# RGenomicsETL/duckhts

Hardware: AMD Instinct MI355X
Metric: read_bam_records_per_sec (higher is better)
Workload: dtype u8

## Files before the change

### duckhts_amd/__init__.py

```python
import ctypes as C
import os

import numpy as np

_HERE = os.path.dirname(os.path.abspath(__file__))
LIB_PATH = os.environ.get("DHTS_LIB") or os.path.join(_HERE, "libduckhts_amd.so")
_LIB = None

BAM_COLUMNS = ["QNAME", "FLAG", "RNAME", "POS", "MAPQ", "CIGAR", "RNEXT", "PNEXT", "TLEN", "SEQ", "QUAL",
               "READ_GROUP_ID", "SAMPLE_ID"]
K_NAMES = ["sigscan", "huff_decode", "lz_resolve", "tiles", "core_unpack", "scan", "string_write", "bcf_check", "bcf_measure", "bcf_write"]


class StrCol(C.Structure):
    _fields_ = [("off", C.c_void_p), ("len", C.c_void_p), ("bytes", C.c_void_p), ("nbytes", C.c_uint64)]


class BamBatch(C.Structure):
    _fields_ = [("n_rows", C.c_int64), ("status", C.c_int32), ("seq_packed", C.c_int32),
                ("flag", C.c_void_p), ("pos", C.c_void_p), ("mapq", C.c_void_p), ("pnext", C.c_void_p),
                ("tlen", C.c_void_p), ("tid", C.c_void_p), ("mtid", C.c_void_p), ("rg_idx", C.c_void_p),
                ("rg_valid", C.c_void_p),
                ("qname", StrCol), ("cigar", StrCol), ("seq", StrCol), ("qual", StrCol), ("rg", StrCol),
                ("first_rec_uoff", C.c_uint64), ("end_uoff", C.c_uint64), ("n_tag_cols", C.c_int32), ("qual_bits", C.c_int32), ("aux_map", C.c_void_p), ("tag_cols", C.c_void_p),
# ... 139 lines not shown
           "dhts_udf_upload", "dhts_udf_apply", "dhts_udf_result_host_bytes", "dhts_udf_fetch", "dhts_udf_seq_kmers", "dhts_udf_kmers_host_bytes", "dhts_udf_kmers_fetch"]


def lib():
    global _LIB
    if _LIB is None:
        if not os.path.exists(LIB_PATH):
            raise RuntimeError(f"{LIB_PATH} is missing: build it with __graft_entry__.build() (hipcc, gfx950)")
        L = C.CDLL(LIB_PATH)
        L.dhts_create.restype = C.c_void_p
        L.dhts_create.argtypes = [C.c_int]
        L.dhts_destroy.argtypes = [C.c_void_p]
        L.dhts_error.restype = C.c_char_p
        L.dhts_error.argtypes = [C.c_void_p]
        L.dhts_open_path.argtypes = [C.c_void_p, C.c_char_p]
        L.dhts_open_host.argtypes = [C.c_void_p, C.c_void_p, C.c_uint64]
        L.dhts_open_tiled.argtypes = [C.c_void_p, C.c_void_p, C.c_uint64, C.c_void_p, C.c_uint64, C.c_int, C.c_void_p,
                                      C.c_uint64]
        L.dhts_resident_bytes.restype = C.c_uint64
        L.dhts_resident_bytes.argtypes = [C.c_void_p]
        L.dhts_bgzf_index.restype = C.c_int64
        L.dhts_bgzf_index.argtypes = [C.c_void_p]
        L.dhts_bgzf_table.argtypes = [C.c_void_p, C.c_void_p, C.c_void_p, C.c_void_p, C.c_int64]
        L.dhts_bgzf_inflate_to_host.restype = C.c_int64
        L.dhts_bgzf_inflate_to_host.argtypes = [C.c_void_p, C.c_int64, C.c_int64, C.c_void_p, C.c_uint64, C.c_void_p]
        L.dhts_bam_open.argtypes = [C.c_void_p]
        L.dhts_bam_header_get.argtypes = [C.c_void_p, C.POINTER(BamHeader)]
        L.dhts_bam_is_text.argtypes = [C.c_void_p]
        L.dhts_debug_sam_records.restype = C.c_int64
        L.dhts_debug_sam_records.argtypes = [C.c_void_p, C.c_void_p, C.c_uint64, C.POINTER(C.c_int64)]
        L.dhts_debug_fastq_records.restype = C.c_int64
        L.dhts_debug_fastq_records.argtypes = [C.c_void_p, C.c_void_p, C.c_uint64, C.POINTER(C.c_int64)]
        L.dhts_debug_tile_stats.argtypes = [C.c_void_p, C.POINTER(C.c_uint64)]
        L.dhts_bam_set_shard.argtypes = [C.c_void_p, C.c_int, C.c_int]
        L.dhts_bam_set_block_range.argtypes = [C.c_void_p, C.c_int64, C.c_int64, C.c_int]
        L.dhts_shard_cut.argtypes = [C.c_void_p, C.c_int64, C.c_uint64, C.c_int, C.c_int, C.POINTER(C.c_int64), C.POINTER(C.c_int64)]
        L.dhts_bam_rewind.argtypes = [C.c_void_p]
        L.dhts_bam_set_regions.argtypes = [C.c_void_p, C.c_char_p]
        L.dhts_bam_std_tag_info.argtypes = [C.c_int, C.c_char_p, C.c_char_p, C.c_char_p]
        L.dhts_bam_set_tag_columns.argtypes = [C.c_void_p, C.c_void_p, C.c_int32]
        L.dhts_bam_set_aux_map.argtypes = [C.c_void_p, C.c_int, C.c_int]
        L.dhts_bam_build_index.restype = C.c_int64
        L.dhts_bam_build_index.argtypes = [C.c_void_p]
        L.dhts_bam_index_bytes.argtypes = [C.c_void_p, C.c_void_p, C.c_uint64]
        L.dhts_bam_set_overlap_intervals.argtypes = [C.c_void_p, C.c_void_p, C.c_void_p, C.c_void_p, C.c_int64]
        L.dhts_bam_load_index.argtypes = [C.c_void_p, C.c_void_p, C.c_uint64]
        L.dhts_bam_next_batch.argtypes = [C.c_void_p, C.c_int64, C.c_uint32, C.POINTER(BamBatch)]
        L.dhts_memcpy_d2h.argtypes = [C.c_void_p, C.c_void_p, C.c_void_p, C.c_uint64]
        L.dhts_sync.argtypes = [C.c_void_p]
        L.dhts_kernel_time_ms.restype = C.c_double
        L.dhts_kernel_time_ms.argtypes = [C.c_void_p, C.c_int, C.POINTER(C.c_int64)]
        L.dhts_kernel_time_reset.argtypes = [C.c_void_p]
        L.dhts_set_timing.argtypes = [C.c_void_p, C.c_int]
        L.dhts_bcf_open.argtypes = [C.c_void_p, C.c_int]
        L.dhts_bcf_info_get.argtypes = [C.c_void_p, C.POINTER(BcfInfo)]
        L.dhts_bcf_set_projection.argtypes = [C.c_void_p, C.c_void_p, C.c_int32]
        L.dhts_bcf_set_block_range.argtypes = [C.c_void_p, C.c_int64, C.c_int64, C.c_int]
        L.dhts_bcf_rewind.argtypes = [C.c_void_p]
        L.dhts_bcf_set_region.argtypes = [C.c_void_p, C.c_char_p]
        L.dhts_bcf_load_index.argtypes = [C.c_void_p, C.c_void_p, C.c_uint64]
        L.dhts_bcf_next_batch.argtypes = [C.c_void_p, C.c_int64, C.POINTER(BcfBatch)]
        L.dhts_fasta_build_index.restype = C.c_int64
        L.dhts_fasta_build_index.argtypes = [C.c_void_p]
        L.dhts_fasta_index_bytes.argtypes = [C.c_void_p, C.c_void_p, C.c_uint64]
        L.dhts_fasta_gzi_bytes.restype = C.c_int64
        L.dhts_fasta_gzi_bytes.argtypes = [C.c_void_p, C.c_void_p, C.c_uint64]
# ... 153 lines not shown
        coff = np.zeros(n, np.uint64)
        clen = np.zeros(n, np.uint32)
        isize = np.zeros(n, np.uint32)
        st = self.L.dhts_bgzf_table(self.h, coff.ctypes.data, clen.ctypes.data, isize.ctypes.data, n)
        return coff, clen, isize, st

    def bgzf_inflate(self, blk0, nblk, cap):
        out = np.zeros(max(cap, 1), np.uint8)
        st = np.zeros(max(nblk, 1), np.int32)
        n = self._chk(self.L.dhts_bgzf_inflate_to_host(self.h, blk0, nblk, out.ctypes.data, cap, st.ctypes.data))
        return out[:n], st[:nblk]

    def bam_open(self):
        self._chk(self.L.dhts_bam_open(self.h))
        return self.header()

    def bam_is_text(self):
        return self.L.dhts_bam_is_text(self.h)

    def debug_sam_records(self):
        n = C.c_int64(0)
        size = self._chk(self.L.dhts_debug_sam_records(self.h, None, 0, C.byref(n)))
        buf = np.zeros(max(size, 1), np.uint8)
        self._chk(self.L.dhts_debug_sam_records(self.h, buf.ctypes.data, size, C.byref(n)))
        return buf[:size].tobytes(), n.value

    TILE_STATS = ("repaired_tiles", "repair_rounds", "fallback_batches", "spec_retries", "validate_rejections", "gave_up")

    def debug_tile_stats(self):
        out = (C.c_uint64 * 8)()
        self._chk(self.L.dhts_debug_tile_stats(self.h, out))
        return {k: int(out[i]) for i, k in enumerate(self.TILE_STATS)}

    def debug_fastq_records(self):
        n = C.c_int64(0)
        size = self._chk(self.L.dhts_debug_fastq_records(self.h, None, 0, C.byref(n)))
        buf = np.zeros(max(size, 1), np.uint8)
        self._chk(self.L.dhts_debug_fastq_records(self.h, buf.ctypes.data, size, C.byref(n)))
        return buf[:size].tobytes(), n.value

    def debug_deflate_codes(self, counts, maxbits):
        cnt = np.ascontiguousarray(counts, dtype=np.uint32)
        assert cnt.ndim == 2
        lens, codes = np.zeros(cnt.shape, np.uint8), np.zeros(cnt.shape, np.uint32)
        f = self.L.dhts_debug_deflate_codes
        f.argtypes = [C.c_void_p, C.c_void_p, C.c_uint32, C.c_uint32, C.c_int64, C.c_void_p, C.c_void_p]
        self._chk(f(self.h, cnt.ctypes.data, cnt.shape[1], maxbits, cnt.shape[0], lens.ctypes.data, codes.ctypes.data))
        return lens, codes

    def header(self):
        h = BamHeader()
        self._chk(self.L.dhts_bam_header_get(self.h, C.byref(h)))
        return {
            "n_ref": h.n_ref,
            "ref_names": [h.ref_name[i] for i in range(h.n_ref)],
            "ref_len": [h.ref_len[i] for i in range(h.n_ref)],
            "text": C.string_at(h.text, h.l_text) if h.l_text else b"",
            "rg_id": [h.rg_id[i] for i in range(h.n_rg)],
            "rg_sm": [h.rg_sm[i] for i in range(h.n_rg)],
            "first_rec_uoff": h.first_rec_uoff,
        }

    def set_shard(self, rank, world):
        self._chk(self.L.dhts_bam_set_shard(self.h, rank, world))

    def set_block_range(self, b0, b1, speculative):
# ... 1404 lines not shown
```

### duckhts_amd/csrc/bam_tiles_lds.hip

```cpp
#pragma once

#ifndef TL_TILE
#define TL_TILE 8192u
#endif
#define TL_RECS (TL_TILE / 32u)
#define TL_HALO 1024u
#define TR_F_ROWS 1ull
#define TR_F_HEAP 2ull
#define TR_F_TIMEOUT 4ull

struct GSrc {
    typedef uint64_t off;
    const uint8_t *g;
    static __device__ __forceinline__ uint64_t none() { return NONE64; }
    __device__ __forceinline__ uint64_t lim(const BamStream &st) const { return st.ulen; }
    __device__ __forceinline__ uint64_t abs(uint64_t o) const { return o; }
    __device__ __forceinline__ uint8_t u8(uint64_t o) const { return g[o]; }
    __device__ __forceinline__ uint32_t u32(uint64_t o) const { return ldu32(g + o); }
    __device__ __forceinline__ uint64_t u64(uint64_t o) const { uint64_t v; __builtin_memcpy(&v, g + o, 8); return v; }
};
struct LSrc { const uint8_t *g; const uint8_t *l; uint64_t base; uint32_t len; };

struct PSrc {
    typedef uint64_t off;
// ... 283 lines not shown
            while (rel < lim) {
                if (rel + 4u > win) { general = true; break; }
                uint32_t v; __builtin_memcpy(&v, buf + rel, 4);
                const int32_t b = (int32_t)__builtin_amdgcn_readfirstlane((int)v);
                if (b < 32) { err = 1; break; }
                if (left - rel - 4u < (uint32_t)b) { if (st.final_batch) err = 1; break; }
                if (lane == 0 && cnt < TL_RECS) rl[cnt] = (uint16_t)rel;
                cnt++; rel += 4u + (uint32_t)b;
            }
#endif
            o = tb + rel;
            if (general && err == 0) {
                while (o < te) {
                    uint32_t bl = 0;
                    const int rc = ((o - tb) + 64 <= (uint64_t)s.len) ? rec_hop_uniform(st, ls, o, lane, bl) : rec_hop(st, gs, o, bl);
                    if (rc == REC_INCOMPLETE) { if (st.final_batch && o < st.ulen) err = 1; break; }
                    if (rc == REC_INVALID) { err = 1; break; }
                    if (lane == 0 && cnt < TL_RECS) rl[cnt] = (uint16_t)(o - tb);
                    cnt++; o += 4ull + bl;
                }
            }
        }
        en = o;
    } else if (first != NONE64) en = first;
    if (lane == 0) {
        out.first[t] = (first != NONE64 && first < te) ? first : NONE64;
        out.end_next[t] = en; out.count[t] = cnt; out.err[t] = err;
        tile_recs_first[t] = (first != NONE64 && first < te) ? first : NONE64;
    }
    __syncthreads();
    for (uint32_t k = lane; k < cnt && k < TL_RECS; k += 64) tile_recs[(size_t)t * TL_RECS + k] = rl[k];
}

extern "C" __global__ void __launch_bounds__(64)
bam_spec_next(BamStream st, uint64_t from, SpecSkip sk, uint64_t *out) {
    const int lane = threadIdx.x;
    GSrc gs; gs.g = st.u;
    uint64_t first = NONE64;
    for (uint64_t base = from & ~63ull; base < st.ulen; base += 64) {
        const uint64_t o = base + (uint64_t)lane;
        bool ok = false;
        if (o < st.ulen && o >= from) {
            RecInfo r;
            if (rec_check_t(st, gs, o, r, false) == REC_OK) {
                ok = true;
                uint64_t o2 = o + 4ull + r.block_len;
                for (int k = 0; k < 2 && ok; k++) {
                    RecInfo r2;
                    const int rc = rec_check_t(st, gs, o2, r2, false);
                    if (rc == REC_INVALID) ok = false;
                    else if (rc == REC_INCOMPLETE) break;
                    else o2 += 4ull + r2.block_len;
                }
                if (ok && spec_skipped(sk, o)) ok = false;
            }
        }
        const uint64_t m = __ballot(ok);
        if (m) { first = base + (uint64_t)(__ffsll((unsigned long long)m) - 1); break; }
    }
    if (lane == 0) *out = first;
}

struct DictG { const uint32_t *off; const uint8_t *bytes; int32_t n; };
struct DictL { const uint32_t *off; const uint8_t *bytes; int32_t n; };
#define RGL_N 32
#define RGL_BYTES 256
// ... 412 lines not shown
```

### duckhts_amd/csrc/dhts_api.hip

```cpp
#include "../../include/duckhts_amd.h"
#include "bgzf_inflate.hip"
#include "bgzf_huff_wave.hip"
#include "bam_records.hip"
#include "bam_tiles_lds.hip"
#include "bam_tile_rows.hip"
#include "bcf_records.hip"
#include "vcf_text.hip"
#include "bed_text.hip"
#include "tabix_text.hip"
#include "sam_text.hip"
#include "fastq_text.hip"
#include "fasta_index.hip"
#include "fasta_nuc.hip"
#include "seq_udf.hip"
#include "bam_bins.hip"
#include "bam_bedcov.hip"
#include "gzip_serial.hip"
#include "bam_tags.hip"
#include "bgzf_deflate.hip"
#include "hts_index.hip"
#include "bcf_header.h"

#include <errno.h>
#include <time.h>
// ... 191 lines not shown
    uint32_t s_patch_cap = 0;
    int64_t s_last_nrec = 0; uint64_t s_last_len = 0;
    int fastq = 0;
    FastaState fa;
    BedState bed;
    NucState nuc;
    BinsState bins;
    BedcovState cov;
    UdfState udf;
    TabixState tbx;
    bool text_any = false;
    DevBuf f_len, f_flag, f_psum, f_rank, f_mark, f_next, f_plus, f_exit, f_entry, f_stop, f_isstart, f_recrank, f_recline;
    DevBuf v_pos_hi;
    DevBuf v_keep, v_endsv; uint64_t proj_gen = 1, keep_gen = 0; int32_t keep_none = 0, fmt_none = 0; bool keep_all = true, fmt_keep_all = true; DevBuf v_fkeep;
    DevBuf v_cnt, v_base, v_line_off, v_rec_len, v_out, v_ctr, v_undef, v_patch, vd_ctg_off, vd_ctg_bytes, vd_ctg_id, vd_id_off, vd_id_bytes, vd_id_id, vd_id_typ, vd_id_ftyp, vd_ctg_hash, vd_id_hash, v_tok_off, v_tok_bytes, v_tok_bits;
    uint32_t v_undef_cap = 65536, v_patch_cap = 1u << 20;
    uint32_t vd_ctg_hmask = 0, vd_id_hmask = 0;
    bool cache_hit = false; std::string pending_tag;
    std::thread stager; StageProg *prog = nullptr; bool growing = false; uint64_t stage_total = 0;
    uint64_t debug_full_len = 0; bool debug_prefix = false;
    DevBuf spec_skip[SPEC_LISTS];
    uint64_t tile_stats[8] = {0, 0, 0, 0, 0, 0, 0, 0};
    int64_t n_blocks = 0; int bgzf_status = 0;
    DevBuf coff, clen, isize, uoff, blk_status;
    std::vector<uint64_t> h_coff, h_uoff; std::vector<uint32_t> h_clen, h_isize;
    DevBuf lit, tok, meta;
    DevBuf stg_lit, stg_tok, wave_ctr;
    DevBuf wg_lit[2], wg_tok[2], stg2_lit, stg2_tok;
    DevBuf blk_off; bool huff_packed = false;
    int64_t isize_repaired = 0;
    bool pool_full_pending = false;
    int64_t pool_per_block = 65536 + 4096;
    DevBuf sg_cnt, sg_base, sg_cand, sg_hits;
    std::vector<uint8_t> built_index; DevBuf ix_end; BamStream last_stream;
    bool ov_active = false; int64_t ov_n = 0;
    DevBuf ov_beg, ov_end, ov_pmax, ov_bmax, ov_id, ov_first, ov_cnt, ov_off, ov_ids;
    int64_t huff_b0 = 0, huff_nb = 0;
    int64_t wave_slots = 0;
    int64_t super_blocks = 524288;
    DevBuf ubuf[2]; int ucur = 0; uint64_t carry_len = 0;
    DevBuf t_first, t_end, t_count, t_err, t_rowbase, d_res, d_nfixed, d_bstat, t_recs, t_recs_first;
    DevBuf t2_first, t2_end, t2_count, t2_err;
    DevBuf t_look; int64_t rows_slots = 0, rows_hint = 0; uint64_t heap_hint[5] = {0, 0, 0, 0, 0};
    DevBuf c_rgflag;
    DevBuf rec_off, c_flag, c_pos, c_mapq, c_pnext, c_tlen, c_tid, c_mtid, c_rgidx, c_rgvalid;
    DevBuf l_qname, l_cigar, l_seq, l_qual, l_rg, cig_rel, ncig_eff, rg_rel, alen_qual;
    DevBuf o_qname, o_cigar, o_seq, o_qual, o_rg, scan_partial, scan_total;
    DevBuf a_qname, a_cigar, a_seq, a_qual, a_rg;
    bool bam_open = false;
    std::vector<std::string> ref_name; std::vector<const char *> ref_name_p; std::vector<uint32_t> ref_len;
    std::string text;
    std::vector<std::string> rg_id, rg_sm; std::vector<char> rg_has_sm; std::vector<const char *> rg_id_p, rg_sm_p;
    uint64_t first_rec_uoff = 0;
    DevBuf d_rg_off, d_rg_bytes;
    std::vector<int32_t> tag_sel; std::vector<dhts_col> tag_out;
    bool aux_on = false, aux_excl_std = false; dhts_aux_map aux_out;
    DevBuf x_excl, x_valid, x_le, x_lp, x_oe, x_op, x_key, x_kind, x_sub, x_payoff, x_payload;
    DevBuf t_codes, t_dir, t_lens, t_offs, t_partial, t_total, t_coldev, t_fixed, t_valid, t_var;
    bool rg_active = false, rg_all = false, rg_nocoor = false;
    std::vector<int64_t> rg_beg, rg_end; std::vector<uint32_t> rg_tid_first;
    DevBuf d_rg_beg, d_rg_end, d_rg_first, c_keep, c_rowmap;
    bool rg_empty_window = false;
    struct ScanWin { int64_t b0, b1; uint64_t first_uoff, end_uoff; };
    std::vector<ScanWin> wins; size_t win_cur = 0; uint64_t scan_end_uoff = ~0ull;
    uint64_t scan_first_uoff = 0;
    bool bcf_open = false; bool bcf_tidy_req = false;
    dhts::BcfHeader bh; dhts::BcfSchema bsch;
// ... 115 lines not shown
        const bool cclean = hipStreamSynchronize(c->copy_stream) == hipSuccess;
        std::lock_guard<std::mutex> lk(g_cs_mu);
        static bool cs_at_exit = false;
        if (!cs_at_exit) { cs_at_exit = true; std::atexit([]() { std::lock_guard<std::mutex> lk2(g_cs_mu); for (auto &x : g_cs) { if (hipSetDevice(x.dev) != hipSuccess) continue; for (int k = 0; k < 2; k++) { (void)hipEventDestroy(x.snap[k]); (void)hipEventDestroy(x.done[k]); } (void)hipStreamDestroy(x.s); } g_cs.clear(); }); }
        if (cclean && g_cs.size() < 32) g_cs.push_back({c->device, c->copy_stream, {c->ev_snap[0], c->ev_snap[1]}, {c->ev_done[0], c->ev_done[1]}});
        else { for (int k = 0; k < 2; k++) { (void)hipEventDestroy(c->ev_snap[k]); (void)hipEventDestroy(c->ev_done[k]); } (void)hipStreamDestroy(c->copy_stream); }
        c->copy_stream = nullptr;
    }
    bool kept = false;
    if (clean) {
        std::lock_guard<std::mutex> lk(g_ss_mu);
        static bool at_exit = false;
        if (!at_exit) { at_exit = true; std::atexit([]() { std::lock_guard<std::mutex> lk2(g_ss_mu); for (auto &x : g_ss) { if (hipSetDevice(x.dev) != hipSuccess) continue; (void)hipEventDestroy(x.ev); (void)hipStreamDestroy(x.sb); (void)hipStreamDestroy(x.s); } g_ss.clear(); }); }
        if (g_ss.size() < 32) { g_ss.push_back({c->device, c->stream, c->stream_b, c->pf_done}); kept = true; }
    }
    if (!kept) { (void)hipEventDestroy(c->pf_done); (void)hipStreamDestroy(c->stream_b); (void)hipStreamDestroy(c->stream); }
    delete c;
}

const char *dhts_error(const dhts_ctx *c) { return c ? c->err.c_str() : "no context (no MI355X device or code object)"; }

static void stop_stager(dhts_ctx *c) {
    if (c->prog && c->stager.joinable()) c->prog->cancel.store(true);
    if (c->stager.joinable()) c->stager.join();
    if (c->prog && !c->pending_tag.empty() && c->prog->finished && c->prog->rc == 0 && c->prog->frontier == c->prog->len) { c->comp.tag = c->pending_tag; c->comp.tag_len = c->prog->len; }
    c->pending_tag.clear();
    delete c->prog; c->prog = nullptr; c->growing = false;
}
static void reset_file_state(dhts_ctx *c) {
    stop_stager(c);
    c->huff_b0 = c->huff_nb = 0; c->file_off = 0; c->file_size = 0; c->seg_split = 0; c->seg_file_off = 0; c->partial_tail = false; c->segs.clear(); c->cache_hit = false; c->gz_plain = c->gz_error = false; c->gz_len = 0; c->plain_text = false; c->vcf_text = false; c->sam_text = false; c->fastq = 0; c->fa.text_ready = false; c->nuc.open = false; c->bins.open = false; c->cov.open = false; c->text_any = false; c->bed.open = false; c->tbx.open = false;
    c->n_blocks = 0; c->bgzf_status = 0; c->bam_open = false; c->range_cut = false; c->last_batch_rows = -1; c->carry_len = 0; c->next_block = 0; c->stream_done = false; c->first_batch = true;
    memset(c->tile_stats, 0, sizeof(c->tile_stats));
    c->h_coff.clear(); c->h_clen.clear(); c->h_isize.clear(); c->h_uoff.clear();
}

int dhts_open_host(dhts_ctx *c, const void *bytes, uint64_t n) {
    if (c) discard_prefetch(c);
    if (!c) return -1;
    HIPCHK(c, hipSetDevice(c->device));
    reset_file_state(c);
    ENSURE(c, c->comp, n + PAD_BYTES);
    HIPCHK(c, hipMemcpyAsync(c->comp.p, bytes, n, hipMemcpyHostToDevice, c->stream));
    HIPCHK(c, hipMemsetAsync((uint8_t *)c->comp.p + n, 0, PAD_BYTES, c->stream));
    HIPCHK(c, hipStreamSynchronize(c->stream));
    c->comp_len = n;
    return 0;
}

int dhts_open_tiled(dhts_ctx *c, const void *head, uint64_t n_head, const void *body, uint64_t n_body, int reps, const void *tail, uint64_t n_tail) {
    if (c) discard_prefetch(c);
    if (!c) return -1;
    HIPCHK(c, hipSetDevice(c->device));
    reset_file_state(c);
    uint64_t n = n_head + n_body * (uint64_t)reps + n_tail;
    ENSURE(c, c->comp, n + PAD_BYTES);
    uint8_t *d = (uint8_t *)c->comp.p;
    if (n_head) HIPCHK(c, hipMemcpyAsync(d, head, n_head, hipMemcpyHostToDevice, c->stream));
    if (n_body && reps > 0) {
        HIPCHK(c, hipMemcpyAsync(d + n_head, body, n_body, hipMemcpyHostToDevice, c->stream));
        for (int r = 1; r < reps; r++) HIPCHK(c, hipMemcpyAsync(d + n_head + n_body * (uint64_t)r, d + n_head, n_body, hipMemcpyDeviceToDevice, c->stream));
    }
    if (n_tail) HIPCHK(c, hipMemcpyAsync(d + n_head + n_body * (uint64_t)reps, tail, n_tail, hipMemcpyHostToDevice, c->stream));
    HIPCHK(c, hipMemsetAsync(d + n, 0, PAD_BYTES, c->stream));
    HIPCHK(c, hipStreamSynchronize(c->stream));
    c->comp_len = n;
// ... 26 lines not shown
```

### duckhts_amd/csrc/dhts_bam_scan.inc

```
struct Batch {
    int64_t b0 = 0, nb = 0; bool in_halo = false, last_of_stream = false, sharded_tail = false, final_batch = false;
    uint64_t carry = 0, ulen = 0, out_base = 0; uint8_t *u = nullptr; int blk_err = 0;
    bool status_pending = false;
};
static const uint32_t NONE32 = 0xffffffffu;
static int batch_begin(dhts_ctx *c, int64_t max_blocks, Batch &B, bool defer = false) {
    if (max_blocks <= 0) max_blocks = 16384;
    if (max_blocks > 24576) max_blocks = 24576;
    B.sharded_tail = (c->shard_b1 < c->n_blocks);
    int64_t b0 = c->next_block;
    int64_t limit = c->shard_b1;
    bool in_halo = b0 >= c->shard_b1;
    if (in_halo) limit = c->n_blocks;
    int64_t nb = limit - b0; if (nb > max_blocks) nb = max_blocks;
    if (in_halo && nb > 4) nb = 4;
    if (nb < 0) nb = 0;
    if (c->first_batch && c->shard_rank != 0 && !in_halo) {
        while (b0 + nb < limit && c->h_uoff[b0 + nb] - c->h_uoff[b0] < (1u << 20) && nb < 24576) nb++;
    }
    B.b0 = b0; B.nb = nb; B.in_halo = in_halo;
    B.last_of_stream = (b0 + nb >= c->n_blocks) && !c->growing;
    {
        const int64_t ahead0 = c->shard_b1 + 8 < c->n_blocks ? c->shard_b1 + 8 : c->n_blocks;
        if (!(c->pf.valid && c->pf.b0 == b0 && c->pf.nb == nb) && huff_ensure(c, b0, nb, ahead0)) return -1;
// ... 192 lines not shown
        int32_t status = 0;
        if (batch_end(c, B, carry_start, false, false, &status)) return -1;
        if (status == 1) break;
        if (status < 0) { rc = -1; err = "the BGZF stream ended on an error"; break; }
    }
    discard_prefetch(c);
    c->next_block = 0; c->carry_len = 0; c->stream_done = false; c->first_batch = true; c->ucur = 0;
    if (rc) return fail(c, "tabix_index: %s", err.c_str());
    if (!inited) init_index();
    uint64_t fin = c->comp_len;
    for (int64_t k = nb; k > 0 && c->h_isize[k - 1] == 0; k--) fin = c->h_coff[k - 1];
    if (!ib.finish(fin << 16)) return fail(c, "tabix_index: %s", ib.err.c_str());
    {
        const uint32_t conf[6] = {(uint32_t)preset, (uint32_t)sc, (uint32_t)bc, (uint32_t)ec, (uint32_t)meta_char, (uint32_t)line_skip}; uint32_t l_nm = 0;
        for (auto &x : names) l_nm += (uint32_t)x.size() + 1;
        auto w32 = [&](uint32_t x) { for (int k = 0; k < 4; k++) ib.aux.push_back((uint8_t)(x >> (8 * k))); };
        for (uint32_t x : conf) w32(x);
        w32(l_nm);
        for (auto &x : names) { ib.aux.insert(ib.aux.end(), x.begin(), x.end()); ib.aux.push_back(0); }
    }
    ib.save(c->built_index);
    return (int64_t)c->built_index.size();
}

extern "C" int dhts_debug_tile_stats(dhts_ctx *c, uint64_t out[8]) {
    if (!c || !out) return -1;
    memcpy(out, c->tile_stats, sizeof(c->tile_stats));
    return 0;
}

static bool rows_deferred_on() { static const bool on = !(getenv("DHTS_ROWS") && !strcmp(getenv("DHTS_ROWS"), "sync")); return on; }
static bool rows_fused_on() { static const bool on = getenv("DHTS_ROWS") && !strcmp(getenv("DHTS_ROWS"), "fused"); return on; }
static int rows_exp() { static const int e = getenv("DHTS_ROWS_EXP") ? (atoi(getenv("DHTS_ROWS_EXP")) & 2) : 0; return e; }
struct RowsQueued { BamCols bc; RowsStr so; };
static int rows_queue(dhts_ctx *c, const BamStream &st, int64_t ntiles, const TileOut &to, uint32_t colmask, RowsQueued &rq) {
    const uint64_t ulen = st.ulen;
    int64_t rcap = (int64_t)(ulen / 160) + 4096; if (c->rows_hint > rcap) rcap = c->rows_hint;
    const uint64_t guess[5] = {ulen / 8 + 65536, ulen / 16 + 65536, ulen / 2 + 65536, ulen / 2 + 65536, ulen / 16 + 65536};
    const uint32_t str_cols = (1u << DHTS_BAM_QNAME) | (1u << DHTS_BAM_CIGAR) | (1u << DHTS_BAM_SEQ) | (1u << DHTS_BAM_QUAL) | (1u << DHTS_BAM_READ_GROUP_ID);
    const bool strings = (colmask & str_cols) != 0;
    const uint32_t hbit[5] = {1u << DHTS_BAM_QNAME, 1u << DHTS_BAM_CIGAR, 1u << DHTS_BAM_SEQ, 1u << DHTS_BAM_QUAL, 1u << DHTS_BAM_READ_GROUP_ID};
    RowsCaps caps; caps.rows = rcap;
    DevBuf *arena[5] = {&c->a_qname, &c->a_cigar, &c->a_seq, &c->a_qual, &c->a_rg};
    for (int k = 0; k < 5; k++) {
        uint64_t want = 0;
        if (colmask & hbit[k]) { want = guess[k]; if (c->heap_hint[k] > want) want = c->heap_hint[k]; }
        if (want) { ENSURE(c, *arena[k], want + PAD_BYTES); caps.heap[k] = arena[k]->cap - PAD_BYTES; } else caps.heap[k] = 0;
    }
    const size_t n = (size_t)rcap;
    ENSURE(c, c->rec_off, n * 4 + 16); ENSURE(c, c->c_rgflag, n + 64);
    ENSURE(c, c->c_flag, n * 2 + 16); ENSURE(c, c->c_pos, n * 8); ENSURE(c, c->c_mapq, n * 4); ENSURE(c, c->c_pnext, n * 8); ENSURE(c, c->c_tlen, n * 8);
    ENSURE(c, c->c_tid, n * 4); ENSURE(c, c->c_mtid, n * 4); ENSURE(c, c->c_rgidx, n * 4); ENSURE(c, c->c_rgvalid, (n / 64 + 2) * 8);
    ENSURE(c, c->l_qname, n * 4 + 16); ENSURE(c, c->l_cigar, n * 4 + 16); ENSURE(c, c->l_seq, n * 4 + 16); ENSURE(c, c->l_qual, n * 4 + 16); ENSURE(c, c->l_rg, n * 4 + 16);
    ENSURE(c, c->cig_rel, n * 4); ENSURE(c, c->ncig_eff, n * 4); ENSURE(c, c->rg_rel, n * 4); ENSURE(c, c->alen_qual, n * 4);
    ENSURE(c, c->o_qname, (n + 1) * 4 + 16); ENSURE(c, c->o_cigar, (n + 1) * 4 + 16); ENSURE(c, c->o_seq, (n + 1) * 4 + 16); ENSURE(c, c->o_qual, (n + 1) * 4 + 16); ENSURE(c, c->o_rg, (n + 1) * 4 + 16);
    BamDict dict; dict.n_rg = (int32_t)c->rg_id.size(); dict.rg_off = (const uint32_t *)c->d_rg_off.p; dict.rg_bytes = (const uint8_t *)c->d_rg_bytes.p; { size_t tb_ = 0; for (auto &id_ : c->rg_id) tb_ += id_.size(); dict.n_bytes = (int32_t)tb_; }
    BamCols &bc = rq.bc; memset(&bc, 0, sizeof(bc));
    bc.flag = (uint16_t *)c->c_flag.p; bc.pos = (int64_t *)c->c_pos.p; bc.mapq = (int32_t *)c->c_mapq.p; bc.pnext = (int64_t *)c->c_pnext.p;
    bc.tlen = (int64_t *)c->c_tlen.p; bc.tid = (int32_t *)c->c_tid.p; bc.mtid = (int32_t *)c->c_mtid.p; bc.rg_idx = (int32_t *)c->c_rgidx.p;
    bc.rg_valid = (uint64_t *)c->c_rgvalid.p; bc.len_qname = (uint32_t *)c->l_qname.p; bc.len_cigar = (uint32_t *)c->l_cigar.p; bc.len_seq = (uint32_t *)c->l_seq.p;
    bc.len_qual = (uint32_t *)c->l_qual.p; bc.len_rg = (uint32_t *)c->l_rg.p; bc.cig_rel = (uint32_t *)c->cig_rel.p; bc.ncig_eff = (uint32_t *)c->ncig_eff.p; bc.rg_rel = (uint32_t *)c->rg_rel.p;
    RowsStr &so = rq.so; memset(&so, 0, sizeof(so));
    so.off[0] = (uint32_t *)c->o_qname.p; so.off[1] = (uint32_t *)c->o_cigar.p; so.off[2] = (uint32_t *)c->o_seq.p; so.off[3] = (uint32_t *)c->o_qual.p; so.off[4] = (uint32_t *)c->o_rg.p;
    for (int k = 0; k < 5; k++) so.heap[k] = (uint8_t *)arena[k]->p;
    so.alen_qual = (uint32_t *)c->alen_qual.p;
    if (c->seq_packed && (colmask & (1u << DHTS_BAM_SEQ))) { ENSURE(c, c->seq_chars, n * 4 + 64); so.seq_chars = (uint32_t *)c->seq_chars.p; }
// ... 96 lines not shown
    ENSURE(c, c->t_rowbase, ntiles * 4 + 16); ENSURE(c, c->d_res, 256); ENSURE(c, c->d_nfixed, 64);
    ENSURE(c, c->t_recs, (size_t)ntiles * TL_RECS * 2 + 64); ENSURE(c, c->t_recs_first, ntiles * 8 + 64);
    ENSURE(c, c->t2_first, ntiles * 8); ENSURE(c, c->t2_end, ntiles * 8); ENSURE(c, c->t2_count, ntiles * 4); ENSURE(c, c->t2_err, ntiles * 4);
    TileOut to; to.first = (uint64_t *)c->t_first.p; to.end_next = (uint64_t *)c->t_end.p; to.count = (uint32_t *)c->t_count.p; to.err = (int32_t *)c->t_err.p;
    TileOut to2; to2.first = (uint64_t *)c->t2_first.p; to2.end_next = (uint64_t *)c->t2_end.p; to2.count = (uint32_t *)c->t2_count.p; to2.err = (int32_t *)c->t2_err.p;
    uint64_t start0;
    if (c->sam_text) start0 = 0;
    else if (c->first_batch) start0 = (c->shard_rank == 0) ? c->scan_first_uoff - out_base : NONE64;
    else start0 = 0;
    if (!c->sam_text && c->first_batch && c->shard_rank == 0 && c->scan_first_uoff < out_base) return fail(c, "internal: header beyond first batch");
    uint64_t res[4] = {0, 0, 0, 0};
    uint64_t first0 = NONE64;
    const bool speculative = (start0 == NONE64);
    const bool fused = !speculative && !(c->rg_active && !c->rg_all) && !(sharded_tail && out_base + ulen > c->h_uoff[c->shard_b1]) && rows_deferred_on();
    unsigned long long hres[16] = {0}; RowsQueued rq;
    uint64_t spec_from = 0, en0 = NONE64; int spec_tries = 0; bool restoring = false;
    SpecSkip sk; memset(&sk, 0, sizeof(sk));
    int status_attempt = 0;
    for (;;) {
        uint64_t start_eff = start0;
        if (speculative && !restoring && spec_tries > 0) {
            uint64_t *d_cand = (uint64_t *)c->d_nfixed.p + 2, cand = NONE64;
            hipLaunchKernelGGL(bam_spec_next, dim3(1), dim3(64), 0, c->stream, st, spec_from, sk, d_cand);
            HIPCHK(c, hipMemcpyAsync(&cand, d_cand, 8, hipMemcpyDeviceToHost, c->stream));
            HIPCHK(c, hipStreamSynchronize(c->stream));
            if (cand == NONE64) { spec_from = 0; restoring = true; c->tile_stats[DHTS_TS_GAVE_UP]++; }
            else { start_eff = cand; c->tile_stats[DHTS_TS_RETRIES]++; }
        }
        to.first = (uint64_t *)c->t_first.p; to.end_next = (uint64_t *)c->t_end.p; to.count = (uint32_t *)c->t_count.p; to.err = (int32_t *)c->t_err.p;
        to2.first = (uint64_t *)c->t2_first.p; to2.end_next = (uint64_t *)c->t2_end.p; to2.count = (uint32_t *)c->t2_count.p; to2.err = (int32_t *)c->t2_err.p;
        uint32_t nfh[2] = {0, 0}, bst[4] = {NONE32, 0, NONE32, 0};
        {
            KTimer tm(c, DHTS_K_TILES);
            hipLaunchKernelGGL(bam_tile_scan, dim3((unsigned)ntiles), dim3(64), 0, c->stream, st, start_eff, ntiles, to, (uint16_t *)c->t_recs.p, (uint64_t *)c->t_recs_first.p, spec_from);
            uint32_t *nf = (uint32_t *)c->d_nfixed.p;
            (void)hipMemsetAsync(nf, 0, 8, c->stream);
            for (int r = 0; r < 2; r++) {
                hipLaunchKernelGGL(bam_tile_fix, dim3((unsigned)((ntiles + 255) / 256)), dim3(256), 0, c->stream, st, TILE_BYTES, ntiles, to, to2, nf + r);
                TileOut tmp = to; to = to2; to2 = tmp;
            }
            hipLaunchKernelGGL(bam_tile_finalize, dim3(1), dim3(1024), 0, c->stream, ntiles, to, (uint32_t *)c->t_rowbase.p, (uint64_t *)c->d_res.p);
        }
        if (fused) { if (rows_queue(c, st, ntiles, to, colmask, rq)) return -1; HIPCHK(c, hipMemcpyAsync(hres, c->d_res.p, 128, hipMemcpyDeviceToHost, c->stream)); }
        HIPCHK(c, hipMemcpyAsync(res, c->d_res.p, 32, hipMemcpyDeviceToHost, c->stream));
        HIPCHK(c, hipMemcpyAsync(&first0, to.first, 8, hipMemcpyDeviceToHost, c->stream));
        if (speculative) HIPCHK(c, hipMemcpyAsync(&en0, to.end_next, 8, hipMemcpyDeviceToHost, c->stream));
        HIPCHK(c, hipMemcpyAsync(nfh, c->d_nfixed.p, 8, hipMemcpyDeviceToHost, c->stream));
        if (B.status_pending) HIPCHK(c, hipMemcpyAsync(bst, c->d_bstat.p, 16, hipMemcpyDeviceToHost, c->stream));
        HIPCHK(c, hipStreamSynchronize(c->stream));
        if (B.status_pending) {
            const int rs = batch_status_resolve(c, B, bst, status_attempt++);
            if (rs < 0) return -1;
            if (rs > 0) {
                ulen = B.ulen; final_batch = B.final_batch;
                st.ulen = ulen; st.final_batch = final_batch ? 1 : 0; c->last_stream = st;
                ntiles = (int64_t)((ulen + TILE_BYTES - 1) / TILE_BYTES); if (ntiles < 1) ntiles = 1;
                spec_from = 0; spec_tries = 0; restoring = false; sk.lists = 0;
                continue;
            }
        }
        if (g_debug) fprintf(stderr, "[dhts] tiles=%lld nfixed=%u,%u\n", (long long)ntiles, nfh[0], nfh[1]);
        c->tile_stats[DHTS_TS_REPAIRED] += (uint64_t)nfh[0] + nfh[1]; c->tile_stats[DHTS_TS_ROUNDS] += (nfh[0] != 0) + (nfh[1] != 0);
        if (nfh[1] != 0) {
            KTimer tm(c, DHTS_K_TILES);
            int rounds = 2; bool seq_fallback = false;
            for (;;) {
                (void)hipMemsetAsync(c->d_nfixed.p, 0, 4, c->stream);
// ... 285 lines not shown
```

### duckhts_amd/csrc/dhts_regions.inc

```
static long long parse_decimal_sep(const char *str, const char **strend) {
    unsigned long long n = 0; int digits = 0, decimals = 0, e = 0; char sign = '+', esign = '+';
    const char *s = str;
    while (*s == ' ' || (*s >= '\t' && *s <= '\r')) s++;
    if (*s == '+' || *s == '-') sign = *s++;
    while (*s) { if (*s >= '0' && *s <= '9') { digits++; n = n * 10 + (unsigned)(*s++ - '0'); } else if (*s == ',') s++; else break; }
    if (*s == '.') { s++; while (*s >= '0' && *s <= '9') { decimals++; digits++; n = n * 10 + (unsigned)(*s++ - '0'); } }
    switch (*s) {
    case 'e': case 'E': s++; if (*s == '+' || *s == '-') esign = *s++; while (*s >= '0' && *s <= '9') e = e * 10 + (*s++ - '0'); if (esign == '-') e = -e; break;
    case 'k': case 'K': e += 3; s++; break;
    case 'm': case 'M': e += 6; s++; break;
    case 'g': case 'G': e += 9; s++; break;
    }
    e -= decimals;
    while (e > 0) { n *= 10; e--; }
    while (e < 0) { n /= 10; e++; }
    *strend = digits > 0 ? s : str;
    return sign == '+' ? (long long)n : -(long long)n;
}

static bool parse_region_token_fn(const std::function<int(const std::string &)> &getid, const std::string &tok, int &tid, int64_t &beg, int64_t &end);
static bool parse_region_token(const std::vector<std::string> &names, const std::string &tok, int &tid, int64_t &beg, int64_t &end) {
    return parse_region_token_fn([&](const std::string &nm) -> int { for (size_t i = 0; i < names.size(); i++) if (names[i] == nm) return (int)i; return -1; }, tok, tid, beg, end);
}
static bool parse_region_token_fn(const std::function<int(const std::string &)> &getid, const std::string &tok, int &tid, int64_t &beg, int64_t &end) {
// ... 360 lines not shown
        all.any = true;
        for (auto &x : merged_windows(w, true)) all.chunks.push_back(x);
    }
    (void)dhts_bcf_set_region(c, nullptr);
    if (whole) return 0;
    std::vector<std::pair<uint64_t, uint64_t>> sg;
    if (all.any) {
        std::sort(all.chunks.begin(), all.chunks.end());
        std::vector<std::pair<uint64_t, uint64_t>> mg;
        const uint64_t gap_bytes = (uint64_t)(getenv("DHTS_WINDOW_GAP_MB") ? atof(getenv("DHTS_WINDOW_GAP_MB")) : 32.0) * (1u << 20);
        for (auto &x : all.chunks) {
            if (!mg.empty() && (x.first >> 16) <= (mg.back().second >> 16) + gap_bytes) { if (x.second > mg.back().second) mg.back().second = x.second; }
            else mg.push_back(x);
        }
        for (auto &x : mg) sg.push_back({x.first >> 16, x.second >> 16});
    }
    *count = (int64_t)sg.size();
    if ((int64_t)sg.size() > cap) { *count = -1; return 0; }
    for (size_t k = 0; k < sg.size(); k++) { beg[k] = sg[k].first; end[k] = sg[k].second; }
    return 0;
}

static void enter_window(dhts_ctx *c, size_t k) {
    const dhts_ctx::ScanWin &w = c->wins[k];
    c->win_cur = k; c->shard_b0 = w.b0; c->shard_b1 = w.b1; c->shard_rank = 0; c->shard_world = (w.b1 < c->n_blocks) ? 2 : 1;
    c->scan_first_uoff = w.first_uoff; c->scan_end_uoff = w.end_uoff;
}
int dhts_bam_rewind(dhts_ctx *c) {
    if (!c) return -1;
    discard_prefetch(c);
    if (!c->wins.empty()) enter_window(c, 0);
    c->next_block = c->shard_b0; c->carry_len = 0; c->stream_done = c->rg_empty_window; c->first_batch = true; c->ucur = 0;
    c->huff_b0 = c->huff_nb = 0;
    memset(c->tile_stats, 0, sizeof(c->tile_stats));
    skip_header_blocks(c);
    return 0;
}
```

### include/duckhts_amd_debug.h

```cpp
#ifndef DUCKHTS_AMD_DEBUG_H
#define DUCKHTS_AMD_DEBUG_H
#include "duckhts_amd.h"
#ifdef __cplusplus
extern "C" {
#endif

void dhts_debug_malloc_stats(uint64_t *calls, uint64_t *bytes, double *seconds);
int64_t dhts_debug_index_prefix(dhts_ctx *, uint64_t nbytes);
int64_t dhts_debug_vcf_records(dhts_ctx *, uint8_t *dst, uint64_t cap, uint32_t *rec_off, int64_t nrec);
int64_t dhts_debug_sam_records(dhts_ctx *, uint8_t *dst, uint64_t cap, int64_t *nrec);
int64_t dhts_debug_fastq_records(dhts_ctx *, uint8_t *dst, uint64_t cap, int64_t *nrec);
int64_t dhts_debug_bed_walk(dhts_ctx *, double *ms_line_table, double *ms_walk);
void dhts_debug_bedcov_max_rows(uint64_t n);
double dhts_debug_time_huff(dhts_ctx *, int64_t b0, int64_t nb, int reps);
double dhts_debug_time_lz(dhts_ctx *, int64_t b0, int64_t nb, int reps);
int dhts_debug_huff_run(dhts_ctx *, int64_t b0, int64_t nb, int kernel);
int dhts_debug_scratch_get(dhts_ctx *, int64_t s, uint32_t *meta4, uint8_t *lit, uint32_t *tok);
int dhts_debug_meta(dhts_ctx *, int64_t s, uint32_t *out4);
int dhts_debug_deflate_codes(dhts_ctx *, const uint32_t *counts, uint32_t nsym, uint32_t maxbits, int64_t ncases, uint8_t *lens_out, uint32_t *codes_out);
int dhts_debug_tile_stats(dhts_ctx *, uint64_t out[8]);
int dhts_debug_diag(dhts_ctx *, unsigned long long *out8);
int dhts_debug_hw_diag(dhts_ctx *, unsigned long long *out16, int reset);
int dhts_debug_tr_diag(dhts_ctx *, unsigned long long *out16, int reset);

#ifdef __cplusplus
}
#endif
#endif
```

Baseline: 614.6 million.

## Add one-thread-per-tile BAM tile scan kernel for large batches

Adds a tile scan kernel that gives each 8 KiB tile to a single lane instead of a full 64-lane wavefront. The lane streams 128-byte lines into registers and builds bitmask prefilters over four byte phases to find candidate record starts, then confirms them with a three-record speculative check. The original wave kernel still handles tile 0, and the new kernel is chosen automatically only when a batch has at least 32640 tiles, with an environment override. It aims to cut the wavefront launch and synchronisation overhead per tile on very large batches, at the cost of per-lane serial work and register pressure. A debug entry point for comparing the two kernels is also added.

Measured after the change: 646.6 million (median of 6 runs). +5.2%, better.

```diff
diff --git a/duckhts_amd/__init__.py b/duckhts_amd/__init__.py
--- a/duckhts_amd/__init__.py
+++ b/duckhts_amd/__init__.py
@@ -195,6 +195,9 @@
         L.dhts_debug_fastq_records.restype = C.c_int64
         L.dhts_debug_fastq_records.argtypes = [C.c_void_p, C.c_void_p, C.c_uint64, C.POINTER(C.c_int64)]
         L.dhts_debug_tile_stats.argtypes = [C.c_void_p, C.POINTER(C.c_uint64)]
+        if hasattr(L, "dhts_debug_tile_scan"):
+            L.dhts_debug_tile_scan.argtypes = [C.c_void_p, C.c_int] + [C.c_void_p] * 6 + [C.c_int64]
+            L.dhts_debug_tile_scan.restype = C.c_int64
         L.dhts_bam_set_shard.argtypes = [C.c_void_p, C.c_int, C.c_int]
         L.dhts_bam_set_block_range.argtypes = [C.c_void_p, C.c_int64, C.c_int64, C.c_int]
         L.dhts_shard_cut.argtypes = [C.c_void_p, C.c_int64, C.c_uint64, C.c_int, C.c_int, C.POINTER(C.c_int64), C.POINTER(C.c_int64)]
@@ -414,6 +417,14 @@
         self._chk(self.L.dhts_debug_tile_stats(self.h, out))
         return {k: int(out[i]) for i, k in enumerate(self.TILE_STATS)}
 
+    def debug_tile_scan(self, kernel, ulen):
+        import numpy as np
+        cap = max(1, (int(ulen) + 8191) // 8192)
+        t = {"first": np.zeros(cap, np.uint64), "end_next": np.zeros(cap, np.uint64), "count": np.zeros(cap, np.uint32), "err": np.zeros(cap, np.int32),
+             "recs_first": np.zeros(cap, np.uint64), "recs": np.zeros((cap, 256), np.uint16)}
+        n = self._chk(self.L.dhts_debug_tile_scan(self.h, {"wave": 0, "lanes": 1}[kernel], *[t[k].ctypes.data for k in ("first", "end_next", "count", "err", "recs_first", "recs")], cap))
+        return {k: v[:n] for k, v in t.items()}
+
     def debug_fastq_records(self):
         n = C.c_int64(0)
         size = self._chk(self.L.dhts_debug_fastq_records(self.h, None, 0, C.byref(n)))
diff --git a/duckhts_amd/csrc/bam_tiles_lds.hip b/duckhts_amd/csrc/bam_tiles_lds.hip
--- a/duckhts_amd/csrc/bam_tiles_lds.hip
+++ b/duckhts_amd/csrc/bam_tiles_lds.hip
@@ -339,6 +339,103 @@
     for (uint32_t k = lane; k < cnt && k < TL_RECS; k += 64) tile_recs[(size_t)t * TL_RECS + k] = rl[k];
 }
 
+#define LS_LINE 128u
+#ifdef __HIP_DEVICE_COMPILE__
+#define LS_X(D, q, r) ((r) == 0 ? (D)[(q)] : (uint32_t)__builtin_amdgcn_alignbyte((D)[(q) + 1], (D)[(q)], (r)))
+#else
+#define LS_X(D, q, r) ((r) == 0 ? (D)[(q)] : (uint32_t)(((((uint64_t)(D)[(q) + 1]) << 32) | (uint64_t)(D)[(q)]) >> (8 * (r))))
+#endif
+__device__ __forceinline__ void lane_line_load(const uint8_t *src, uint32_t k0, uint32_t pad, uint4 (&v)[8]) {
+#pragma unroll
+    for (uint32_t i = 0; i < 8; i++) { const uint32_t k = k0 + 16u * i; v[i] = *(const uint4 *)(src + (k < pad ? k : 0u)); }
+}
+__device__ __forceinline__ void lane_prefilter(const uint32_t (&D)[39], uint32_t n_ref1, uint32_t (&S)[4]) {
+#pragma unroll
+    for (uint32_t r = 0; r < 4; r++) {
+        uint64_t mb = 0, mr = 0, ms = 0, mq = 0;
+#pragma unroll
+        for (uint32_t q = 0; q < 38; q++) {
+            const uint32_t x = LS_X(D, q, r);
+            if (q < 32) mb |= (uint64_t)((int32_t)x >= 32) << q;
+            if (q >= 1) mr |= (uint64_t)(x + 1u < n_ref1) << q;
+            if (q >= 3 && q < 35) mq |= (uint64_t)((x & 0xffu) != 0u) << q;
+            if (q >= 5 && q < 37) ms |= (uint64_t)((int32_t)x >= 0) << q;
+        }
+        S[r] = (uint32_t)(mb & (mr >> 1) & (mq >> 3) & (ms >> 5) & (mr >> 6));
+    }
+}
+__device__ __forceinline__ bool lane_spec3(const BamStream &st, const GSrc &gs, uint64_t o) {
+    RecInfo r;
+    if (rec_check_t(st, gs, o, r, false) != REC_OK) return false;
+    uint64_t o2 = o + 4ull + r.block_len;
+    for (int k = 0; k < 2; k++) {
+        RecInfo r2;
+        const int rc = rec_check_t(st, gs, o2, r2, false);
+        if (rc == REC_INVALID) return false;
+        if (rc == REC_INCOMPLETE) break;
+        o2 += 4ull + r2.block_len;
+    }
+    return true;
+}
+__device__ __forceinline__ void tile_scan_lane(const BamStream &st, int64_t t, const TileOut &out, uint16_t *tile_recs, uint64_t *tile_recs_first) {
+    const uint64_t tb = (uint64_t)t * TL_TILE;
+    if (tb >= st.ulen) return;
+    const uint64_t left64 = st.ulen - tb;
+    const uint32_t left = left64 > 0xffffffffull ? 0xffffffffu : (uint32_t)left64;
+    const uint32_t lim = left < TL_TILE ? left : TL_TILE;
+    const uint32_t avail = left < TL_TILE + TL_HALO ? left : TL_TILE + TL_HALO;
+    const uint32_t pad = (avail + 15u) & ~15u;
+    const uint8_t *src = st.u + tb;
+    GSrc gs; gs.g = st.u;
+    const uint32_t n_ref1 = (uint32_t)st.n_ref + 1u;
+    uint32_t first = 0xffffffffu;
+    uint4 cur[8], nxt[8];
+    lane_line_load(src, 0u, pad, cur);
+    for (uint32_t lb = 0; lb < lim && first == 0xffffffffu; lb += LS_LINE) {
+        lane_line_load(src, lb + LS_LINE, pad, nxt);
+        uint32_t D[39], S[4];
+#pragma unroll
+        for (uint32_t i = 0; i < 8; i++) { D[4 * i] = cur[i].x; D[4 * i + 1] = cur[i].y; D[4 * i + 2] = cur[i].z; D[4 * i + 3] = cur[i].w; }
+        D[32] = nxt[0].x; D[33] = nxt[0].y; D[34] = nxt[0].z; D[35] = nxt[0].w; D[36] = nxt[1].x; D[37] = nxt[1].y; D[38] = nxt[1].z;
+        lane_prefilter(D, n_ref1, S);
+        uint32_t any = S[0] | S[1] | S[2] | S[3];
+        while (any != 0u && first == 0xffffffffu) {
+            const uint32_t q = (uint32_t)__ffs((int)any) - 1u;
+            any &= any - 1u;
+            uint32_t ph = ((S[0] >> q) & 1u) | (((S[1] >> q) & 1u) << 1) | (((S[2] >> q) & 1u) << 2) | (((S[3] >> q) & 1u) << 3);
+            while (ph != 0u && first == 0xffffffffu) {
+                const uint32_t rel = lb + 4u * q + ((uint32_t)__ffs((int)ph) - 1u);
+                ph &= ph - 1u;
+                if (rel < lim && lane_spec3(st, gs, tb + rel)) first = rel;
+            }
+        }
+#pragma unroll
+        for (uint32_t i = 0; i < 8; i++) cur[i] = nxt[i];
+    }
+    uint64_t en = NONE64; uint32_t cnt = 0; int err = 0;
+    if (first != 0xffffffffu) {
+        uint32_t rel = first;
+        while (rel < lim) {
+            if (left - rel < 4u) { if (st.final_batch) err = 1; break; }
+            const int32_t b = (int32_t)ldu32(src + rel);
+            if (b < 32) { err = 1; break; }
+            if (left - rel - 4u < (uint32_t)b) { if (st.final_batch) err = 1; break; }
+            if (cnt < TL_RECS) tile_recs[(size_t)t * TL_RECS + cnt] = (uint16_t)rel;
+            cnt++; rel += 4u + (uint32_t)b;
+        }
+        en = tb + rel;
+    }
+    const uint64_t f = first != 0xffffffffu ? tb + first : NONE64;
+    out.first[t] = f; out.end_next[t] = en; out.count[t] = cnt; out.err[t] = err;
+    tile_recs_first[t] = f;
+}
+extern "C" __global__ void __launch_bounds__(64)
+bam_tile_scan_lanes(BamStream st, int64_t ntiles, TileOut out, uint16_t *tile_recs, uint64_t *tile_recs_first) {
+    const int64_t t = 1 + (int64_t)blockIdx.x * 64 + threadIdx.x;
+    if (t >= ntiles) return;
+    tile_scan_lane(st, t, out, tile_recs, tile_recs_first);
+}
+
 extern "C" __global__ void __launch_bounds__(64)
 bam_spec_next(BamStream st, uint64_t from, SpecSkip sk, uint64_t *out) {
     const int lane = threadIdx.x;
diff --git a/duckhts_amd/csrc/dhts_api.hip b/duckhts_amd/csrc/dhts_api.hip
--- a/duckhts_amd/csrc/dhts_api.hip
+++ b/duckhts_amd/csrc/dhts_api.hip
@@ -247,7 +247,7 @@
     bool pool_full_pending = false;
     int64_t pool_per_block = 65536 + 4096;
     DevBuf sg_cnt, sg_base, sg_cand, sg_hits;
-    std::vector<uint8_t> built_index; DevBuf ix_end; BamStream last_stream;
+    std::vector<uint8_t> built_index; DevBuf ix_end; BamStream last_stream{};
     bool ov_active = false; int64_t ov_n = 0;
     DevBuf ov_beg, ov_end, ov_pmax, ov_bmax, ov_id, ov_first, ov_cnt, ov_off, ov_ids;
     int64_t huff_b0 = 0, huff_nb = 0;
@@ -429,6 +429,7 @@
     c->huff_b0 = c->huff_nb = 0; c->file_off = 0; c->file_size = 0; c->seg_split = 0; c->seg_file_off = 0; c->partial_tail = false; c->segs.clear(); c->cache_hit = false; c->gz_plain = c->gz_error = false; c->gz_len = 0; c->plain_text = false; c->vcf_text = false; c->sam_text = false; c->fastq = 0; c->fa.text_ready = false; c->nuc.open = false; c->bins.open = false; c->cov.open = false; c->text_any = false; c->bed.open = false; c->tbx.open = false;
     c->n_blocks = 0; c->bgzf_status = 0; c->bam_open = false; c->range_cut = false; c->last_batch_rows = -1; c->carry_len = 0; c->next_block = 0; c->stream_done = false; c->first_batch = true;
     memset(c->tile_stats, 0, sizeof(c->tile_stats));
+    c->last_stream = BamStream{};
     c->h_coff.clear(); c->h_clen.clear(); c->h_isize.clear(); c->h_uoff.clear();
 }
 
diff --git a/duckhts_amd/csrc/dhts_bam_scan.inc b/duckhts_amd/csrc/dhts_bam_scan.inc
--- a/duckhts_amd/csrc/dhts_bam_scan.inc
+++ b/duckhts_amd/csrc/dhts_bam_scan.inc
@@ -248,6 +248,51 @@
 static bool rows_deferred_on() { static const bool on = !(getenv("DHTS_ROWS") && !strcmp(getenv("DHTS_ROWS"), "sync")); return on; }
 static bool rows_fused_on() { static const bool on = getenv("DHTS_ROWS") && !strcmp(getenv("DHTS_ROWS"), "fused"); return on; }
 static int rows_exp() { static const int e = getenv("DHTS_ROWS_EXP") ? (atoi(getenv("DHTS_ROWS_EXP")) & 2) : 0; return e; }
+#define TILE_SCAN_LANES_MIN 32640
+static int tile_scan_mode() {
+    const char *e = getenv("DHTS_TILE_SCAN");
+    if (!e || !strcmp(e, "auto")) return 0;
+    if (!strcmp(e, "wave")) return 1;
+    if (!strcmp(e, "lanes")) return 2;
+    static std::atomic<bool> warned{false};
+    if (!warned.exchange(true)) fprintf(stderr, "[dhts] DHTS_TILE_SCAN=%s is not wave, lanes or auto: using auto\n", e);
+    return 0;
+}
+static bool tile_scan_lanes_on(int64_t ntiles) { const int m = tile_scan_mode(); return m == 2 || (m == 0 && ntiles >= TILE_SCAN_LANES_MIN); }
+static void tile_scan_launch(dhts_ctx *c, bool lanes, const BamStream &st, uint64_t start0, int64_t ntiles, const TileOut &to, uint16_t *recs, uint64_t *recs_first, uint64_t spec_from) {
+    if (lanes && ntiles > 1) {
+        hipLaunchKernelGGL(bam_tile_scan, dim3(1), dim3(64), 0, c->stream, st, start0, ntiles, to, recs, recs_first, spec_from);
+        hipLaunchKernelGGL(bam_tile_scan_lanes, dim3((unsigned)((ntiles - 1 + 63) / 64)), dim3(64), 0, c->stream, st, ntiles, to, recs, recs_first);
+    } else
+        hipLaunchKernelGGL(bam_tile_scan, dim3((unsigned)ntiles), dim3(64), 0, c->stream, st, start0, ntiles, to, recs, recs_first, spec_from);
+}
+extern "C" int64_t dhts_debug_tile_scan(dhts_ctx *c, int kernel, uint64_t *first, uint64_t *end_next, uint32_t *count, int32_t *err, uint64_t *recs_first,
+                                        uint16_t *recs, int64_t ntiles_cap) {
+    if (!c) return -1;
+    if (kernel != 0 && kernel != 1) return fail(c, "dhts_debug_tile_scan: kernel is 0 (wave) or 1 (lanes)");
+    const BamStream st = c->last_stream;
+    if (!st.u) return fail(c, "dhts_debug_tile_scan: no batch has been read");
+    HIPCHK(c, hipSetDevice(c->device));
+    int64_t ntiles = (int64_t)((st.ulen + TILE_BYTES - 1) / TILE_BYTES); if (ntiles < 1) ntiles = 1;
+    if (ntiles > ntiles_cap) return fail(c, "dhts_debug_tile_scan: the tables are too small");
+    DevBuf d_first, d_end, d_count, d_err, d_rf, d_recs;
+    ENSURE(c, d_first, ntiles * 8); ENSURE(c, d_end, ntiles * 8); ENSURE(c, d_count, ntiles * 4); ENSURE(c, d_err, ntiles * 4);
+    ENSURE(c, d_rf, ntiles * 8 + 64); ENSURE(c, d_recs, (size_t)ntiles * TL_RECS * 2 + 64);
+    HIPCHK(c, hipMemsetAsync(d_first.p, 0xee, ntiles * 8, c->stream)); HIPCHK(c, hipMemsetAsync(d_end.p, 0xee, ntiles * 8, c->stream));
+    HIPCHK(c, hipMemsetAsync(d_count.p, 0xee, ntiles * 4, c->stream)); HIPCHK(c, hipMemsetAsync(d_err.p, 0xee, ntiles * 4, c->stream));
+    HIPCHK(c, hipMemsetAsync(d_rf.p, 0xee, ntiles * 8, c->stream)); HIPCHK(c, hipMemsetAsync(d_recs.p, 0xee, (size_t)ntiles * TL_RECS * 2, c->stream));
+    TileOut to; to.first = (uint64_t *)d_first.p; to.end_next = (uint64_t *)d_end.p; to.count = (uint32_t *)d_count.p; to.err = (int32_t *)d_err.p;
+    tile_scan_launch(c, kernel == 1, st, 0, ntiles, to, (uint16_t *)d_recs.p, (uint64_t *)d_rf.p, 0);
+    HIPCHK(c, hipGetLastError());
+    if (first) HIPCHK(c, hipMemcpyAsync(first, d_first.p, ntiles * 8, hipMemcpyDeviceToHost, c->stream));
+    if (end_next) HIPCHK(c, hipMemcpyAsync(end_next, d_end.p, ntiles * 8, hipMemcpyDeviceToHost, c->stream));
+    if (count) HIPCHK(c, hipMemcpyAsync(count, d_count.p, ntiles * 4, hipMemcpyDeviceToHost, c->stream));
+    if (err) HIPCHK(c, hipMemcpyAsync(err, d_err.p, ntiles * 4, hipMemcpyDeviceToHost, c->stream));
+    if (recs_first) HIPCHK(c, hipMemcpyAsync(recs_first, d_rf.p, ntiles * 8, hipMemcpyDeviceToHost, c->stream));
+    if (recs) HIPCHK(c, hipMemcpyAsync(recs, d_recs.p, (size_t)ntiles * TL_RECS * 2, hipMemcpyDeviceToHost, c->stream));
+    HIPCHK(c, hipStreamSynchronize(c->stream));
+    return ntiles;
+}
 struct RowsQueued { BamCols bc; RowsStr so; };
 static int rows_queue(dhts_ctx *c, const BamStream &st, int64_t ntiles, const TileOut &to, uint32_t colmask, RowsQueued &rq) {
     const uint64_t ulen = st.ulen;
@@ -410,7 +455,7 @@
         uint32_t nfh[2] = {0, 0}, bst[4] = {NONE32, 0, NONE32, 0};
         {
             KTimer tm(c, DHTS_K_TILES);
-            hipLaunchKernelGGL(bam_tile_scan, dim3((unsigned)ntiles), dim3(64), 0, c->stream, st, start_eff, ntiles, to, (uint16_t *)c->t_recs.p, (uint64_t *)c->t_recs_first.p, spec_from);
+            tile_scan_launch(c, tile_scan_lanes_on(ntiles), st, start_eff, ntiles, to, (uint16_t *)c->t_recs.p, (uint64_t *)c->t_recs_first.p, spec_from);
             uint32_t *nf = (uint32_t *)c->d_nfixed.p;
             (void)hipMemsetAsync(nf, 0, 8, c->stream);
             for (int r = 0; r < 2; r++) {
diff --git a/duckhts_amd/csrc/dhts_regions.inc b/duckhts_amd/csrc/dhts_regions.inc
--- a/duckhts_amd/csrc/dhts_regions.inc
+++ b/duckhts_amd/csrc/dhts_regions.inc
@@ -416,6 +416,7 @@
     if (!c->wins.empty()) enter_window(c, 0);
     c->next_block = c->shard_b0; c->carry_len = 0; c->stream_done = c->rg_empty_window; c->first_batch = true; c->ucur = 0;
     c->huff_b0 = c->huff_nb = 0;
+    c->last_stream = BamStream{};
     memset(c->tile_stats, 0, sizeof(c->tile_stats));
     skip_header_blocks(c);
     return 0;
diff --git a/include/duckhts_amd_debug.h b/include/duckhts_amd_debug.h
--- a/include/duckhts_amd_debug.h
+++ b/include/duckhts_amd_debug.h
@@ -19,6 +19,8 @@
 int dhts_debug_meta(dhts_ctx *, int64_t s, uint32_t *out4);
 int dhts_debug_deflate_codes(dhts_ctx *, const uint32_t *counts, uint32_t nsym, uint32_t maxbits, int64_t ncases, uint8_t *lens_out, uint32_t *codes_out);
 int dhts_debug_tile_stats(dhts_ctx *, uint64_t out[8]);
+int64_t dhts_debug_tile_scan(dhts_ctx *, int kernel, uint64_t *first, uint64_t *end_next, uint32_t *count, int32_t *err, uint64_t *recs_first,
+                             uint16_t *recs, int64_t ntiles_cap);
 int dhts_debug_diag(dhts_ctx *, unsigned long long *out8);
 int dhts_debug_hw_diag(dhts_ctx *, unsigned long long *out16, int reset);
 int dhts_debug_tr_diag(dhts_ctx *, unsigned long long *out16, int reset);
```
